# timlod/onset-fingerprinting

Hardware: AMD Instinct MI355X
Metric: frames/sec (1024-pt, hop 256, 48 kHz) detect+FFT+classify at 1/2/4/8 MI355X (higher is better)
Workload: dtype f32

## Files before the change

### include/onsetfp.h

```cpp
#ifndef ONSETFP_H
#define ONSETFP_H

#include <stdint.h>

#ifdef __cplusplus
extern "C" {
#endif

#define OFP_OK 0
#define OFP_ERR_INVALID 1
#define OFP_ERR_HIP 2
#define OFP_ERR_NODEVICE 3
#define OFP_ERR_WORKSPACE 4
#define OFP_ERR_NOCONVERGE 5

#define OFP_ABI_VERSION 3

int ofp_abi_version(void);
const char* ofp_last_error(void);
int ofp_device_count(void);
int ofp_device_check(int device, char* buf, int buflen);

#define OFP_RUNTIME_QUEUES_VAR "GPU_MAX_HW_QUEUES"
#define OFP_RUNTIME_QUEUES "16"
// ... 90 lines not shown
    int64_t mm_S;
    int64_t tu;
    int32_t sm_seg;
    int32_t merge;
    int32_t hp_early;
    int32_t hp_staged;
    int32_t hp_spread;
    int32_t hp_lines;
    int32_t ar_sym;
    int32_t ar_through;
    int32_t ar_lines;
    int32_t db_sym;
    int32_t mm_il;
    int32_t mm_through;
    int32_t ar_il;
    int32_t use_sum;
} ofp_detect_plan;
int ofp_detect_plan_query(const ofp_detector* det, int64_t n_clips, int64_t n_samples, int64_t warm, int want_rel,
                          const void* d_rel, ofp_detect_plan* out);
int ofp_detect_plan_for(const ofp_detector_params* p, const ofp_detect_tuning* t, int n_cus, int64_t n_clips,
                        int64_t n_samples, int64_t warm, int want_rel, const void* d_rel, ofp_detect_plan* out);

enum {
    OFP_CANON_LOG10 = 0,
    OFP_CANON_EXP10 = 1,
    OFP_CANON_RECT_DB = 2,
    OFP_CANON_REL_LINEAR = 3,
    OFP_CANON_AR_STEP = 4,
    OFP_CANON_MIN_STEP = 5,
    OFP_CANON_MAX_STEP = 6
};
int ofp_canon_eval(int32_t op, const float* d_x, const float* d_y, int64_t n, float p0, float p1, float p2, float* d_out,
                   void* stream);

#define OFP_DETECT_INFO_LEN 16
int ofp_detect_offline(ofp_detector* det, const float* d_x, int64_t n_clips, int64_t n_samples,
                       int64_t warm, float* d_rel, ofp_onset* d_records, int64_t cap_per_clip,
                       int64_t* d_counts, void* d_ws, int64_t ws_bytes, int64_t* h_info,
                       void* stream);

int ofp_detect_offline_enqueue(ofp_detector* det, const float* d_x, int64_t n_clips, int64_t n_samples,
                               int64_t warm, float* d_rel, ofp_onset* d_records, int64_t cap_per_clip,
                               int64_t* d_counts, void* d_ws, int64_t ws_bytes, void* stream);
int ofp_detect_offline_complete(ofp_detector* det, const float* d_x, int64_t n_clips, int64_t n_samples,
                                int64_t warm, float* d_rel, ofp_onset* d_records, int64_t cap_per_clip,
                                int64_t* d_counts, void* d_ws, int64_t ws_bytes, int64_t* h_info, void* stream);

int ofp_detect_offline_begin(ofp_detector* det, const float* d_x, int64_t n_clips, int64_t n_samples,
                             int64_t warm, void* d_ws, int64_t ws_bytes, void* stream);
int ofp_detect_offline_finish(ofp_detector* det, const float* d_x, int64_t n_clips, int64_t n_samples,
                              int64_t warm, float* d_rel, ofp_onset* d_records, int64_t cap_per_clip,
                              int64_t* d_counts, void* d_ws, int64_t ws_bytes, int64_t* h_info, void* stream);

int ofp_detect_offline_finish_enqueue(ofp_detector* det, const float* d_x, int64_t n_clips, int64_t n_samples,
                                      int64_t warm, float* d_rel, ofp_onset* d_records, int64_t cap_per_clip,
                                      int64_t* d_counts, void* d_ws, int64_t ws_bytes, void* stream);

int ofp_detect_offline_begin_input(ofp_detector* det, const float* d_x, int64_t n_clips, int64_t n_samples,
                                   int64_t warm, void* d_ws, int64_t ws_bytes, void* stream);
int ofp_detect_offline_begin_iir(ofp_detector* det, const float* d_x, int64_t n_clips, int64_t n_samples,
                                 int64_t warm, void* d_ws, int64_t ws_bytes, void* stream);
int ofp_pack_records(const ofp_onset* d_records, const int64_t* d_counts, int64_t n_clips, int64_t cap_per_clip,
                     int64_t cap_total, int32_t clip_offset, ofp_onset* d_block, void* stream);

int64_t ofp_stream_state_bytes(const ofp_detector* det);
int ofp_stream_state_init(ofp_detector* det, void* d_state, void* stream);
// ... 519 lines not shown
```

### onset_fingerprinting_amd/_lib.py

```python
import ctypes
import os
import subprocess
from pathlib import Path

_HERE = Path(__file__).resolve().parent
LIB_PATH = _HERE / "libonsetfp.so"


class OnsetFPError(RuntimeError):
    pass


class DetectorParams(ctypes.Structure):
    _fields_ = [
        ("n_channels", ctypes.c_int32),
        ("block_size", ctypes.c_int32),
        ("floor_db", ctypes.c_float),
        ("hp_enabled", ctypes.c_int32),
        ("hp_b", ctypes.c_float * 5),
        ("hp_a", ctypes.c_float * 5),
        ("fast_attack", ctypes.c_float),
        ("fast_release", ctypes.c_float),
        ("slow_attack", ctypes.c_float),
        ("slow_release", ctypes.c_float),
# ... 180 lines not shown
        ("d_audio", ctypes.c_void_p),
        ("audio_len", ctypes.c_int64),
        ("d_starts", ctypes.c_void_p),
        ("n_onsets", ctypes.c_int64),
    ]


_vp, _i32, _i64, _f32, _f64 = ctypes.c_void_p, ctypes.c_int32, ctypes.c_int64, ctypes.c_float, ctypes.c_double
_f32p_h = ctypes.POINTER(ctypes.c_float)
_long_p = ctypes.POINTER(ctypes.c_long)

SIGNATURES = {
    "ofp_abi_version": (ctypes.c_int, []),
    "ofp_last_error": (ctypes.c_char_p, []),
    "ofp_runtime_prepare": (ctypes.c_int, []),
    "ofp_device_count": (ctypes.c_int, []),
    "ofp_device_check": (ctypes.c_int, [ctypes.c_int, ctypes.c_char_p, ctypes.c_int]),
    "ar_envelope": (None, [_f32p_h, _f32p_h, _f32, _f32, ctypes.c_int, ctypes.c_int]),
    "minmax_envelope": (None, [_f32p_h, _f32p_h, _f32p_h, _f32, _f32, _f32, ctypes.c_int, ctypes.c_int]),
    "backtrack_onsets": (None, [_f32p_h, _long_p, _long_p, _f32, _f32, ctypes.c_long, ctypes.c_long,
                                ctypes.c_long, ctypes.c_long]),
    "ofp_lfilter": (ctypes.c_int, [_f32p_h, _f32p_h, _f32p_h, _f32p_h, ctypes.c_int, _f32p_h, ctypes.c_long,
                                   ctypes.c_int]),
    "ofp_detector_create": (ctypes.c_int, [ctypes.POINTER(DetectorParams), ctypes.POINTER(ctypes.c_double),
                                           ctypes.POINTER(ctypes.c_double), ctypes.POINTER(_vp)]),
    "ofp_detector_destroy": (ctypes.c_int, [_vp]),
    "ofp_detector_set_tuning": (ctypes.c_int, [_vp, ctypes.POINTER(DetectTuning)]),
    "ofp_pack_records": (ctypes.c_int, [_vp, _vp, _i64, _i64, _i64, ctypes.c_int32, _vp, _vp]),
    "ofp_detect_workspace_bytes": (_i64, [_vp, _i64, _i64, _i64]),
    "ofp_detect_plan_query": (ctypes.c_int, [_vp, _i64, _i64, _i64, ctypes.c_int, _vp, ctypes.POINTER(DetectPlan)]),
    "ofp_detect_plan_for": (ctypes.c_int, [ctypes.POINTER(DetectorParams), ctypes.POINTER(DetectTuning), ctypes.c_int,
                                           _i64, _i64, _i64, ctypes.c_int, _vp, ctypes.POINTER(DetectPlan)]),
    "ofp_canon_eval": (ctypes.c_int, [_i32, _vp, _vp, _i64, _f32, _f32, _f32, _vp, _vp]),
    "ofp_detect_offline": (ctypes.c_int, [_vp, _vp, _i64, _i64, _i64, _vp, _vp, _i64, _vp, _vp, _i64,
                                          ctypes.POINTER(_i64), _vp]),
    "ofp_detect_offline_enqueue": (ctypes.c_int, [_vp, _vp, _i64, _i64, _i64, _vp, _vp, _i64, _vp, _vp, _i64, _vp]),
    "ofp_detect_offline_complete": (ctypes.c_int, [_vp, _vp, _i64, _i64, _i64, _vp, _vp, _i64, _vp, _vp, _i64,
                                                   ctypes.POINTER(_i64), _vp]),
    "ofp_detect_offline_finish_enqueue": (ctypes.c_int, [_vp, _vp, _i64, _i64, _i64, _vp, _vp, _i64, _vp, _vp, _i64, _vp]),
    "ofp_detect_offline_begin": (ctypes.c_int, [_vp, _vp, _i64, _i64, _i64, _vp, _i64, _vp]),
    "ofp_detect_offline_finish": (ctypes.c_int, [_vp, _vp, _i64, _i64, _i64, _vp, _vp, _i64, _vp, _vp, _i64,
                                                 ctypes.POINTER(_i64), _vp]),
    "ofp_detect_offline_begin_input": (ctypes.c_int, [_vp, _vp, _i64, _i64, _i64, _vp, _i64, _vp]),
    "ofp_detect_offline_begin_iir": (ctypes.c_int, [_vp, _vp, _i64, _i64, _i64, _vp, _i64, _vp]),
    "ofp_stream_state_bytes": (_i64, [_vp]),
    "ofp_stream_state_init": (ctypes.c_int, [_vp, _vp, _vp]),
    "ofp_stream_process": (ctypes.c_int, [_vp, _vp, _vp, _i64, _i64, _i32, _i64, _vp, _vp, _i64, _vp, _vp]),
    "ofp_stream_calibrate": (ctypes.c_int, [_vp, _vp, _vp, _i64, _i64, _i64, _i64, _vp, _vp, _vp]),
    "ofp_detector_set_thresholds": (ctypes.c_int, [_vp, ctypes.POINTER(ctypes.c_double), ctypes.POINTER(ctypes.c_double)]),
    "ofp_stft_power": (ctypes.c_int, [_vp, _i64, _i64, _i32, _i32, _i32, _vp, _vp]),
    "ofp_stft_power_mel": (ctypes.c_int, [_vp, _i64, _i64, _i32, _i32, _i32, _vp, _i32, _vp, _vp, _vp, _vp, _i32, _vp,
                                          _i64, _vp]),
    "ofp_detect_planar_input": (_vp, [_vp, _i64, _i64, _i64, _vp]),
    "ofp_detect_planar_stride": (_i64, [_vp, _i64, _i64, _i64]),
    "ofp_stft_frames": (ctypes.c_int, [_vp, _i64, _i64, _i32, _vp, _vp, _vp, _vp, _vp, _i64, _i32, _i32,
                                       _vp, _vp, _vp]),
    "ofp_extract_frames": (ctypes.c_int, [_vp, _i64, _i32, _vp, _i64, _i32, _vp, _vp]),
    "ofp_mel": (ctypes.c_int, [_vp, _i64, _i32, _i32, _vp, _vp, _vp, _vp, _vp, _vp]),
    "ofp_mfcc": (ctypes.c_int, [_vp, _i64, _i32, _i32, _f32, _f32, _vp, _vp, _vp, _vp]),
    "ofp_dense": (ctypes.c_int, [_vp, _i64, _i32, _i32, _vp, _vp, _vp, _vp, _i32, _vp, _vp]),
    "ofp_mlp_create": (ctypes.c_int, [_i32, ctypes.POINTER(_i32), ctypes.POINTER(_i32), ctypes.POINTER(_vp),
                                      ctypes.POINTER(_vp), ctypes.POINTER(_vp), ctypes.POINTER(_vp),
                                      ctypes.POINTER(_vp)]),
    "ofp_mlp_destroy": (ctypes.c_int, [_vp]),
    "ofp_mlp_lds_bytes": (_i64, [_vp]),
    "ofp_mlp_forward": (ctypes.c_int, [_vp, _vp, _i64, _vp, _vp]),
# ... 263 lines not shown
```

### onset_fingerprinting_amd/csrc/ofp_canon.hip

```cpp
#include "ofp_common.h"
#include "../../include/ofp_math.h"

namespace {

using ofp::cdiv;

struct CanonArgs {
    int32_t op;
    float p0, p1, p2;
};

__global__ __launch_bounds__(256) void k_canon_eval(CanonArgs a, const float* __restrict__ x, const float* __restrict__ y,
                                                    int64_t n, float* __restrict__ out) {
    const int64_t step = (int64_t)gridDim.x * blockDim.x;
    for (int64_t i = (int64_t)blockIdx.x * blockDim.x + threadIdx.x; i < n; i += step) {
        const float xi = x[i];
        float r;
        switch (a.op) {
            case OFP_CANON_LOG10: r = ofp_log10f(xi); break;
            case OFP_CANON_EXP10: r = ofp_exp10f(xi); break;
            case OFP_CANON_RECT_DB: r = ofp_rect_db(xi, a.p0); break;
            case OFP_CANON_REL_LINEAR: r = ofp_rel_linear(xi, a.p0); break;
            case OFP_CANON_AR_STEP: r = ofp_ar_step(xi, y[i], a.p0, a.p1); break;
            case OFP_CANON_MIN_STEP: r = ofp_min_step(xi, y[i], a.p2, a.p0, a.p1); break;
            default: r = ofp_max_step(xi, y[i], a.p2, a.p0); break;
        }
        out[i] = r;
    }
}

}

extern "C" int ofp_canon_eval(int32_t op, const float* d_x, const float* d_y, int64_t n, float p0, float p1, float p2,
                              float* d_out, void* stream) {
    OFP_REQUIRE(op >= OFP_CANON_LOG10 && op <= OFP_CANON_MAX_STEP, "ofp_canon_eval: unknown op %d", (int)op);
    OFP_REQUIRE(n >= 0, "ofp_canon_eval: negative n");
    if (n == 0) return OFP_OK;
    OFP_REQUIRE(d_x && d_out, "ofp_canon_eval: NULL argument");
    const bool two = op >= OFP_CANON_AR_STEP;
    OFP_REQUIRE(!two || d_y, "ofp_canon_eval: op %d takes a second operand, d_y is NULL", (int)op);
    CanonArgs a{op, p0, p1, p2};
    if (op == OFP_CANON_MIN_STEP || op == OFP_CANON_MAX_STEP) a.p2 = ofp_ialpha(p0);
    const unsigned blocks = (unsigned)(cdiv(n, 256) < 8192 ? cdiv(n, 256) : 8192);
    hipLaunchKernelGGL(k_canon_eval, dim3(blocks), dim3(256), 0, (hipStream_t)stream, a, d_x, d_y, n, d_out);
    OFP_LAUNCH_CHECK("k_canon_eval");
    return OFP_OK;
}
```

### onset_fingerprinting_amd/csrc/ofp_detect.hip

```cpp
#include <algorithm>
#include <cstdlib>
#include <cmath>
#include <cstring>
#include <new>
#include <vector>

#include "../../include/ofp_math.h"
#include "ofp_common.h"

#include "ofp_detector.h"

#define OFP_LATENCY_BOUND_KERNEL() __builtin_amdgcn_s_setprio(3)

namespace {

using ofp::align_up;
using ofp::cdiv;

typedef float v2f __attribute__((ext_vector_type(2)));

struct Geom {
    int64_t N;
    int64_t Nm;
    int64_t n_w;
    int64_t n_wb;
    int64_t U;
    int64_t V;
    int64_t Nv;
    int32_t C, B;
};
__host__ __device__ inline int64_t hp_dst(const Geom& g, int64_t v) {
    return v < g.n_wb ? v : (v >= g.n_w ? v - g.n_w + g.n_wb : -1);
}
__host__ __device__ inline int64_t u_src(const Geom& g, int64_t u) { return u < g.n_wb ? u : u - g.n_wb; }
__host__ __device__ inline int64_t u_src_planar(const Geom& g, int64_t u) { return u < g.n_wb ? u : u - g.n_wb + g.n_w; }

template <int PB4, int OUT, bool EV, class F>
__device__ __forceinline__ void walk(const float* ip, float* op, int64_t n, int& rem, F& f) {
    auto one = [&](float x) {
        float o = f(x);
// ... 1651 lines not shown
                if (a.U[a.slot(clip, k, c, r)] == HP_EMPTY) continue;
                const uint32_t* m = a.M + a.mslot(clip, k, c, r, q);
                if (m[0] == z0 && m[1] == z1 && m[2] == z2 && m[3] == z3) {
                    joined = r;
                    break;
                }
            }
            if (joined >= 0) n_done = q + 1;
        }
    }
    if (!act) return;
    if (!whole) {
        if (sb == 0) a.ran[ci] = (int8_t)own;
        a.done[ci * a.S + sb] = 1;
        return;
    }
    if (own < 0 || a.guessed[ci]) {
        uint32_t* u = a.U + a.slot(clip, k, c, a.R);
        uint32_t* e = a.E + a.slot(clip, k, c, a.R);
        const uint32_t* ej = joined >= 0 ? a.E + a.slot(clip, k, c, joined) : nullptr;
#pragma unroll
        for (int i = 0; i < 4; ++i) {
            u[i] = xin[i];
            e[i] = ej ? ej[i] : ofp_f2u(s.z[i]);
        }
    }
    a.ran[ci] = (int8_t)a.R;
    for (int q = 0; q < n_done; ++q) a.done[ci * a.S + q] = 1;
    __threadfence();
    a.mrg[ci] = (int8_t)joined;
    if (joined >= 0) atomicAdd(a.counters + 1, 1);
}

__global__ __launch_bounds__(256) void k_rect_db(Geom g, const float* __restrict__ xt, float* __restrict__ buf,
                                                 int64_t n_chains, int from_x, float floor_db) {
    const int64_t total = n_chains * g.U;
    const int64_t tid0 = (int64_t)blockIdx.x * blockDim.x + threadIdx.x, nthr = (int64_t)gridDim.x * blockDim.x;
    if (!from_x) {
        float4* b4 = reinterpret_cast<float4*>(buf);
        const int64_t n4 = total >> 2;
        for (int64_t i = tid0; i < n4; i += nthr) {
            float4 v = b4[i];
            v.x = ofp_rect_db(v.x, floor_db);
            v.y = ofp_rect_db(v.y, floor_db);
            v.z = ofp_rect_db(v.z, floor_db);
            v.w = ofp_rect_db(v.w, floor_db);
            b4[i] = v;
        }
        for (int64_t i = (n4 << 2) + tid0; i < total; i += nthr) buf[i] = ofp_rect_db(buf[i], floor_db);
        return;
    }
    for (int64_t i = tid0; i < total; i += nthr) {
        const int64_t chain = i / g.U, u = i - chain * g.U;
        buf[i] = ofp_rect_db(xt[chain * g.Nv + u_src_planar(g, u)], floor_db);
    }
}

__global__ __launch_bounds__(64) void k_rect_db_sym(ArArgs a, float* __restrict__ buf, int64_t n_waves,
                                                    double* __restrict__ P) {
    const int64_t id = blockIdx.x;
    if (id >= n_waves) return;
    const int lane = threadIdx.x;
    const int64_t j = id % a.n_chunks;
    const int64_t chain = id / a.n_chunks;
    const int64_t base = j * a.L;
    const int64_t len = min(a.L, a.g.U - base);
    float4* xs = reinterpret_cast<float4*>(buf + chain * a.g.U + base);
    const int64_t ng = len >> 2;
    const double c = (double)a.sa, q = 1.0 - c;
    const double q2 = q * q, q4 = q2 * q2;
    double q256 = q4;
    for (int i = 0; i < 6; ++i) q256 *= q256;
    double w = c;
    for (int i = 0; i < lane; ++i) w *= q4;
    double acc = 0.0;
    auto one = [&](float4 v, int64_t g) {
        v.x = ofp_rect_db(v.x, a.floor_db);
        v.y = ofp_rect_db(v.y, a.floor_db);
        v.z = ofp_rect_db(v.z, a.floor_db);
        v.w = ofp_rect_db(v.w, a.floor_db);
        xs[ng - 1 - g] = v;
        acc += w * ((double)v.w + q * ((double)v.z + q * ((double)v.y + q * (double)v.x)));
        w *= q256;
    };
    int64_t g = lane;
    for (; g + 192 < ng; g += 256) {
        const float4 v0 = xs[ng - 1 - g], v1 = xs[ng - 1 - g - 64], v2 = xs[ng - 1 - g - 128], v3 = xs[ng - 1 - g - 192];
        __builtin_amdgcn_sched_barrier(0);
        one(v0, g);
        one(v1, g + 64);
        one(v2, g + 128);
        one(v3, g + 192);
    }
    for (; g < ng; g += 64) one(xs[ng - 1 - g], g);
    for (int o = 32; o > 0; o >>= 1) acc += __shfl_xor(acc, o);
    if (lane == 0) P[id] = acc;
}

__device__ __forceinline__ void rel_out_tile(const Geom& g, float* __restrict__ buf, float* __restrict__ rel_out,
                                             float floor_db, int TU, uint32_t* __restrict__ sum_max,
                                             uint32_t* __restrict__ sum_minv, int64_t nb, float* __restrict__ rel_warm,
                                             int planar, int64_t tile_x, float* tile) {
    const int C = g.C;
    const int S = TU + 4;
    const int64_t clip = blockIdx.y;
    const int64_t u0 = tile_x * TU;
    const int nt = (int)min<int64_t>(TU, g.U - u0);
    const int total = nt * C;
    const bool sum = sum_max != nullptr && u0 + nt > g.n_wb;
    const int64_t j0 = max<int64_t>(u0 - g.n_wb, 0) / g.B;
    const int nbt = TU / g.B + 2;
    uint32_t* s_max = reinterpret_cast<uint32_t*>(tile + (size_t)C * S);
    uint32_t* s_minv = s_max + C * nbt;
    const int lb = (g.B & (g.B - 1)) == 0 ? 31 - __clz(g.B) : -1;
    const int mbase = (int)(u0 - g.n_wb - j0 * g.B);
    if (sum) {
        for (int i = threadIdx.x; i < 2 * C * nbt; i += 256) s_max[i] = 0u;
        __syncthreads();
    }
    const bool vec = (g.U & 3) == 0 && (TU & 3) == 0 && (nt & 3) == 0 && ((g.n_wb * C) & 3) == 0 &&
                     (((int64_t)TU * C) & 3) == 0 && ((g.Nm * C) & 3) == 0;
    if (vec) {
        const int q = nt >> 2;
        const int lq = (q & (q - 1)) == 0 ? 31 - __clz(q) : -1;
        auto at = [&](int i) -> float4* {
            const int c = lq >= 0 ? i >> lq : i / q, t = (i - c * q) << 2;
            return reinterpret_cast<float4*>(buf + (clip * C + c) * g.U + u0 + t);
        };
        auto one = [&](int i, float4 v) {
            const int c = lq >= 0 ? i >> lq : i / q, t = (i - c * q) << 2;
            v.x = ofp_rel_linear(v.x, floor_db);
            v.y = ofp_rel_linear(v.y, floor_db);
            v.z = ofp_rel_linear(v.z, floor_db);
            v.w = ofp_rel_linear(v.w, floor_db);
            if (planar) *at(i) = v;
            *reinterpret_cast<float4*>(tile + c * S + t) = v;
            const int m = mbase + t;
            if (sum && m >= 0) {
                float hi = fmaxf(fmaxf(v.x, v.y), fmaxf(v.z, v.w)), lo = fminf(fminf(v.x, v.y), fminf(v.z, v.w));
                if (!(hi >= 0.0f)) hi = 0.0f;
                if (!(lo >= 0.0f)) lo = __builtin_inff();
                const int jb = lb >= 0 ? m >> lb : m / g.B;
                atomicMax(&s_max[c * nbt + jb], ofp_f2u(hi));
                atomicMax(&s_minv[c * nbt + jb], 0x7f800000u - ofp_f2u(lo));
            }
        };
        int i = threadIdx.x;
        for (; i + 768 < q * C; i += 1024) {
            const float4 v0 = *at(i), v1 = *at(i + 256), v2 = *at(i + 512), v3 = *at(i + 768);
            __builtin_amdgcn_sched_barrier(0);
            one(i, v0);
            one(i + 256, v1);
            one(i + 512, v2);
            one(i + 768, v3);
        }
        for (; i < q * C; i += 256) one(i, *at(i));
    } else {
        for (int i = threadIdx.x; i < total; i += 256) {
            const int c = i / nt, t = i - c * nt;
            float* p = buf + (clip * C + c) * g.U + u0 + t;
            const float v = ofp_rel_linear(*p, floor_db);
            if (planar) *p = v;
            tile[c * S + t] = v;
        }
    }
    __syncthreads();
    if (sum) {
        for (int i = threadIdx.x; i < C * nbt; i += 256) {
            const int c = i / nbt;
            const int64_t j = j0 + (i - c * nbt);
            if (j < nb && (s_max[i] | s_minv[i]) != 0u) {
                atomicMax(&sum_max[(clip * nb + j) * C + c], s_max[i]);
                atomicMax(&sum_minv[(clip * nb + j) * C + c], s_minv[i]);
            }
        }
    }
    if (!rel_out) return;
    float* dst = rel_out + clip * g.Nm * C;
    float* dstw = rel_warm ? rel_warm + clip * g.n_wb * C : nullptr;
    const int64_t m0 = u0 - g.n_wb;
    if (vec && (m0 >= 0 || m0 + nt <= 0) && (reinterpret_cast<uintptr_t>(rel_out) & 15u) == 0) {
        if (m0 < 0 && !dstw) return;
        float4* d4 = reinterpret_cast<float4*>(m0 < 0 ? dstw + u0 * C : dst + m0 * C);
        const int lc = (C & (C - 1)) == 0 ? 31 - __clz(C) : -1;
        for (int i = threadIdx.x; i < (total >> 2); i += 256) {
            float o[4];
#pragma unroll
            for (int e = 0; e < 4; ++e) {
                const int j = 4 * i + e;
                const int t = lc >= 0 ? j >> lc : j / C, c = j - t * C;
                o[e] = tile[c * S + t];
            }
            d4[i] = make_float4(o[0], o[1], o[2], o[3]);
        }
        return;
    }
    for (int i = threadIdx.x; i < total; i += 256) {
        const int t = i / C, c = i - t * C;
        const int64_t m = u0 + t - g.n_wb;
        if (m >= 0) dst[m * C + c] = tile[c * S + t];
        else if (dstw) dstw[(u0 + t) * C + c] = tile[c * S + t];
    }
}

__global__ __launch_bounds__(256) void k_rel_out(Geom g, float* __restrict__ buf, float* __restrict__ rel_out,
                                                 float floor_db, int TU, uint32_t* __restrict__ sum_max,
                                                 uint32_t* __restrict__ sum_minv, int64_t nb, float* __restrict__ rel_warm,
                                                 int planar, int64_t n_tiles) {
    extern __shared__ float tile[];
    for (int64_t tx = blockIdx.x; tx < n_tiles; tx += gridDim.x) {
        rel_out_tile(g, buf, rel_out, floor_db, TU, sum_max, sum_minv, nb, rel_warm, planar, tx, tile);
        __syncthreads();
    }
}

template <int CH>
__global__ __launch_bounds__(256) void k_rel_out_il(Geom g, float* __restrict__ rel, float* __restrict__ rel_warm, float floor_db,
                                                    uint32_t* __restrict__ sum_max, uint32_t* __restrict__ sum_minv,
                                                    int64_t nb, int64_t n_wu) {
    const int lane = threadIdx.x & 63;
    const int wave = __builtin_amdgcn_readfirstlane(threadIdx.x >> 6);
    const int64_t clip = blockIdx.y;
    const int n4 = g.B * (CH / 4);
    for (int64_t j = (int64_t)blockIdx.x * 4 + wave; j < n_wu + nb; j += (int64_t)gridDim.x * 4) {
        const bool in_main = j >= n_wu;
        float4* const p = in_main ? reinterpret_cast<float4*>(rel + (clip * g.Nm + (j - n_wu) * g.B) * CH)
                               : reinterpret_cast<float4*>(rel_warm + (clip * g.n_wb + j * g.B) * CH);
        float4 hi = make_float4(0.0f, 0.0f, 0.0f, 0.0f);
        const float inf = __builtin_inff();
        float4 lo = make_float4(inf, inf, inf, inf);
        auto one = [&](int i, float4 v) {
            v.x = ofp_rel_linear(v.x, floor_db);
            v.y = ofp_rel_linear(v.y, floor_db);
            v.z = ofp_rel_linear(v.z, floor_db);
            v.w = ofp_rel_linear(v.w, floor_db);
            p[i] = v;
            hi.x = fmaxf(hi.x, v.x); hi.y = fmaxf(hi.y, v.y); hi.z = fmaxf(hi.z, v.z); hi.w = fmaxf(hi.w, v.w);
            lo.x = fminf(lo.x, v.x); lo.y = fminf(lo.y, v.y); lo.z = fminf(lo.z, v.z); lo.w = fminf(lo.w, v.w);
        };
        int i = lane;
        for (; i + 192 < n4; i += 256) {
            const float4 v0 = p[i], v1 = p[i + 64], v2 = p[i + 128], v3 = p[i + 192];
            __builtin_amdgcn_sched_barrier(0);
            one(i, v0);
            one(i + 64, v1);
            one(i + 128, v2);
            one(i + 192, v3);
        }
        for (; i < n4; i += 64) one(i, p[i]);
        if (sum_max == nullptr || !in_main) continue;
#pragma unroll
        for (int o = 32; o >= CH / 4; o >>= 1) {
            hi.x = fmaxf(hi.x, __shfl_xor(hi.x, o)); hi.y = fmaxf(hi.y, __shfl_xor(hi.y, o));
            hi.z = fmaxf(hi.z, __shfl_xor(hi.z, o)); hi.w = fmaxf(hi.w, __shfl_xor(hi.w, o));
            lo.x = fminf(lo.x, __shfl_xor(lo.x, o)); lo.y = fminf(lo.y, __shfl_xor(lo.y, o));
            lo.z = fminf(lo.z, __shfl_xor(lo.z, o)); lo.w = fminf(lo.w, __shfl_xor(lo.w, o));
        }
        if (lane < CH / 4) {
            auto minv = [&](float v) { return 0x7f800000u - ofp_f2u(v >= 0.0f ? v : inf); };
            const int64_t at = (clip * nb + (j - n_wu)) * CH + 4 * lane;
            *reinterpret_cast<uint4*>(sum_max + at) = make_uint4(ofp_f2u(hi.x), ofp_f2u(hi.y), ofp_f2u(hi.z), ofp_f2u(hi.w));
            *reinterpret_cast<uint4*>(sum_minv + at) = make_uint4(minv(lo.x), minv(lo.y), minv(lo.z), minv(lo.w));
        }
    }
}

struct ScanArgs {
    Geom g;
    const float* rel;
    const float* thr_mn;
    const float* thr_mx;
    const float* on_f;
    const float* off_f;
    const double* on_d;
    int manual;
    int64_t nb, n_clips;
    int32_t* first_cross;
    int32_t* last_below;
    uint32_t* vflag;
    const uint32_t* sum_max;
    const uint32_t* sum_minv;
};
// ... 1236 lines not shown
        OFP_HIP(hipStreamSynchronize(c.stream));
        int stuck = 0;
        for (int q = 0; q < G; ++q) {
            stuck = h_flags[2 * q] + h_flags[2 * q + 1];
            rec.info[0] += 1;
            rec.info[3] += stuck;
            if (stuck == 0) break;
        }
        it += G;
        if (stuck == 0) break;
        if (l.max_passes > 0 && it > l.max_passes)
            return ofp::fail(OFP_ERR_NOCONVERGE, "hp stage: %d chains still unresolved after %d rounds", stuck, it);
    }
    return OFP_OK;
}

ArArgs ar_args(const Call& c) {
    const Layout& l = c.l;
    const auto& p = c.d->p;
    ArArgs a;
    a.g = l.g;
    a.xdb = c.xdb; a.dif = c.dif; a.rel = c.a.rel; a.rel_warm = c.rel_warm;
    a.fa = p.fast_attack; a.fr = p.fast_release; a.sa = p.slow_attack; a.sr = p.slow_release; a.floor_db = p.floor_db;
    a.L = l.ar_L; a.W = l.ar_W; a.Wc = l.ar_Wc; a.Wf = l.ar_Wf; a.n_chunks = l.ar_chunks; a.S = l.ar_S;
    a.through = l.ar_through ? 1 : 0; a.lines = l.ar_lines ? 1 : 0;
    return a;
}

int decibels(Call& c) {
    const Layout& l = c.l;
    const auto& p = c.d->p;
    const int64_t chains = c.chains();
    if (l.db_sym) {
        hipLaunchKernelGGL(k_rect_db_sym, dim3((unsigned)(chains * l.ar_chunks)), dim3(64), 0, c.stream, ar_args(c), c.xdb,
                           chains * l.ar_chunks, c.at<double>(l.o_ar_P));
        OFP_LAUNCH_CHECK("k_rect_db_sym");
    } else {
        const unsigned ew_grid = (unsigned)std::min<int64_t>(cdiv(chains * l.g.U, 256), 256 * 16);
        hipLaunchKernelGGL(k_rect_db, dim3(ew_grid), dim3(256), 0, c.stream, l.g, c.xt, c.xdb, chains, p.hp_enabled ? 0 : 1,
                           p.floor_db);
        OFP_LAUNCH_CHECK("k_rect_db");
    }
    return OFP_OK;
}

int followers(Call& c, bool host_verified) {
    const Layout& l = c.l;
    const ArArgs a = ar_args(c);
    const int64_t chains = c.chains();
    const int64_t nt = chains * l.ar_chunks;
    uint32_t* used = c.at<uint32_t>(l.o_ar_state);
    if (l.ar_sym) {
        double* P = c.at<double>(l.o_ar_P);
        if (!l.db_sym) {
            hipLaunchKernelGGL(k_ar_sym_local, dim3((unsigned)nt), dim3(64), 0, c.stream, a, nt, P);
            OFP_LAUNCH_CHECK("k_ar_sym_local");
        }
        hipLaunchKernelGGL(k_ar_sym_combine, dim3((unsigned)chains), dim3(64), 0, c.stream, a, (const double*)P, used);
        OFP_LAUNCH_CHECK("k_ar_sym_combine");
        const int64_t ntg = chains * cdiv(l.ar_chunks, l.ar_S);
        if (l.merge)
            hipLaunchKernelGGL(l.ar_il ? (l.g.C == 8 ? k_ar_warm_both<true, 8> : k_ar_warm_both<true, 4>)
                                       : (l.ar_lines ? k_ar_warm_both<true> : k_ar_warm_both<false>),
                               dim3((unsigned)cdiv(ntg, 64)), dim3(64), 0, c.stream, a, ntg, used, state_arrays(used, 2 * nt).endA);
        else
            hipLaunchKernelGGL(k_ar_warm2, dim3(2 * (unsigned)cdiv(ntg, 64)), dim3(64), 0, c.stream, a, ntg, used);
        OFP_LAUNCH_CHECK("k_ar_warm2");
// ... 581 lines not shown
```

### onset_fingerprinting_amd/detection.py

```python
import ctypes
from typing import Optional

import numpy as np
import torch
from scipy import signal as sig

from . import _lib
from ._lib import DetectorParams, DetectTuning, OnsetFPError, check

ONSET_DTYPE = np.dtype([("clip", np.int32), ("channel", np.int32), ("sample", np.int64)])


def _stream_ptr(device):
    return ctypes.c_void_p(torch.cuda.current_stream(device).cuda_stream)


def _dev(device):
    if isinstance(device, torch.device):
        return device
    return torch.device("cuda", int(device))


def _detector_params(n_signals, block_size, floor, hipass_freq, fast_ar, slow_ar, on_threshold, off_threshold,
                     cooldown, backtrack, backtrack_buffer_size, backtrack_smooth_size, sr):
# ... 209 lines not shown
    if tuning:
        bd.set_tuning(**tuning)
    out = bd.detect(xt.contiguous(), warm=warm, want_rel=want_rel)
    recs = BatchDetector.records_to_numpy(out)
    rel = out["rel"].cpu().numpy() if want_rel else None
    return recs, rel, bd.last_info


def detect_plan(n_signals, n_clips, n_samples, block_size=128, sr=96000, warm=None, want_rel=True, rel_aligned=True,
                tuning=None, n_cus=256, floor=-70.0, hipass_freq=2000.0, fast_ar=(3.0, 383.0), slow_ar=(2205.0, 2205.0),
                on_threshold=0.5, off_threshold=0.1, cooldown=1323, backtrack=False, backtrack_buffer_size=128,
                backtrack_smooth_size=5):
    p, _, _ = _detector_params(n_signals, block_size, floor, hipass_freq, fast_ar, slow_ar, on_threshold, off_threshold,
                               cooldown, backtrack, backtrack_buffer_size, backtrack_smooth_size, sr)
    t = _tuning(tuning or {})
    warm = int(0.5 * sr) if warm is None else int(warm)
    plan = _lib.DetectPlan()
    check(_lib.lib().ofp_detect_plan_for(ctypes.byref(p), ctypes.byref(t), int(n_cus), n_clips, n_samples, warm,
                                         int(bool(want_rel)), None if rel_aligned or not want_rel else 4,
                                         ctypes.byref(plan)), "ofp_detect_plan_for")
    return plan.as_dict()


CANON_OPS = {"log10": 0, "exp10": 1, "rect_db": 2, "rel_linear": 3, "ar_step": 4, "min_step": 5, "max_step": 6}


def canon_eval(op, x, y=None, p0=0.0, p1=0.0, out=None):
    assert x.is_cuda and x.dtype == torch.float32 and x.is_contiguous()
    if y is not None:
        assert y.is_cuda and y.dtype == torch.float32 and y.is_contiguous() and y.numel() == x.numel()
    if out is None:
        out = torch.empty_like(x)
    assert out.is_cuda and out.dtype == torch.float32 and out.is_contiguous() and out.numel() == x.numel()
    check(_lib.lib().ofp_canon_eval(CANON_OPS[op], x.data_ptr(), y.data_ptr() if y is not None else None, x.numel(),
                                    p0, p1, 0.0, out.data_ptr(), _stream_ptr(x.device)), "ofp_canon_eval")
    return out


def group_onsets_device(out, n_channels, max_distance=1000, min_channels=3, close_channel=None, cap_groups=None):
    L = _lib.lib()
    recs, counts = out["records"], out["counts"]
    n_clips, cap = recs.shape[0], recs.shape[1]
    cap_groups = int(cap_groups) if cap_groups is not None else cap
    ws = torch.empty(int(L.ofp_group_workspace_bytes(n_clips, cap)), dtype=torch.uint8, device=recs.device)
    groups = torch.empty((n_clips, cap_groups, n_channels), dtype=torch.int64, device=recs.device)
    n_groups = torch.zeros(n_clips, dtype=torch.int64, device=recs.device)
    check(L.ofp_group_onsets(recs.data_ptr(), cap, counts.data_ptr(), n_clips, n_channels, int(max_distance),
                             int(min_channels), -1 if close_channel is None else int(close_channel),
                             groups.data_ptr(), cap_groups, n_groups.data_ptr(), ws.data_ptr(), ws.numel(),
                             _stream_ptr(recs.device)), "ofp_group_onsets")
    return groups, n_groups


def group_windows_device(x, groups, n_groups, frame_length, pre_samples, use_min_onset=True, cap_total=None):
    if x.dim() == 2:
        x = x.unsqueeze(0)
    assert x.is_cuda and x.dtype == torch.float32 and x.is_contiguous()
    n_clips, N, C = x.shape
    cap_groups = groups.shape[1]
    assert groups.shape == (n_clips, cap_groups, C) and groups.dtype == torch.int64 and groups.is_contiguous()
    cap_total = int(cap_total) if cap_total is not None else n_clips * cap_groups
    windows = torch.empty((cap_total, C, frame_length), dtype=torch.float32, device=x.device)
    offsets = torch.empty(n_clips + 1, dtype=torch.int64, device=x.device)
    check(_lib.lib().ofp_group_windows(x.data_ptr(), n_clips, N, C, groups.data_ptr(), cap_groups, n_groups.data_ptr(),
                                  int(pre_samples), int(bool(use_min_onset)), int(frame_length), windows.data_ptr(),
                                  cap_total, offsets.data_ptr(), _stream_ptr(x.device)), "ofp_group_windows")
# ... 435 lines not shown
```

Measured before the change: 230.5 million.

## Stage log/exp lookup tables in LDS and software-pipeline elementwise dB kernels

Copies the log and exp2 lookup tables into shared memory per block and evaluates rect_db and rel_linear from those copies instead of from global/constant tables. Rewrites the elementwise loops in the rect_db and rel_out kernels with a prefetching helper that loads the next iteration before computing the current one. Also regroups k_rect_db_sym into 256-thread blocks holding four waves each. Adds an LDS-table canon_eval entry point for testing. Each block now pays a table fill and a barrier, and the double-precision polynomial work per element is unchanged.

```diff
diff --git a/include/onsetfp.h b/include/onsetfp.h
--- a/include/onsetfp.h
+++ b/include/onsetfp.h
@@ -146,6 +146,7 @@
 };
 int ofp_canon_eval(int32_t op, const float* d_x, const float* d_y, int64_t n, float p0, float p1, float p2, float* d_out,
                    void* stream);
+int ofp_canon_eval_lds(int32_t op, const float* d_x, int64_t n, float floor_db, float* d_out, void* stream);
 
 #define OFP_DETECT_INFO_LEN 16
 int ofp_detect_offline(ofp_detector* det, const float* d_x, int64_t n_clips, int64_t n_samples,
diff --git a/onset_fingerprinting_amd/_lib.py b/onset_fingerprinting_amd/_lib.py
--- a/onset_fingerprinting_amd/_lib.py
+++ b/onset_fingerprinting_amd/_lib.py
@@ -236,6 +236,7 @@
     "ofp_detect_plan_for": (ctypes.c_int, [ctypes.POINTER(DetectorParams), ctypes.POINTER(DetectTuning), ctypes.c_int,
                                            _i64, _i64, _i64, ctypes.c_int, _vp, ctypes.POINTER(DetectPlan)]),
     "ofp_canon_eval": (ctypes.c_int, [_i32, _vp, _vp, _i64, _f32, _f32, _f32, _vp, _vp]),
+    "ofp_canon_eval_lds": (ctypes.c_int, [_i32, _vp, _i64, _f32, _vp, _vp]),
     "ofp_detect_offline": (ctypes.c_int, [_vp, _vp, _i64, _i64, _i64, _vp, _vp, _i64, _vp, _vp, _i64,
                                           ctypes.POINTER(_i64), _vp]),
     "ofp_detect_offline_enqueue": (ctypes.c_int, [_vp, _vp, _i64, _i64, _i64, _vp, _vp, _i64, _vp, _vp, _i64, _vp]),
diff --git a/onset_fingerprinting_amd/csrc/ofp_canon.hip b/onset_fingerprinting_amd/csrc/ofp_canon.hip
--- a/onset_fingerprinting_amd/csrc/ofp_canon.hip
+++ b/onset_fingerprinting_amd/csrc/ofp_canon.hip
@@ -1,5 +1,6 @@
 #include "ofp_common.h"
 #include "../../include/ofp_math.h"
+#include "ofp_canon_dev.h"
 
 namespace {
 
@@ -29,6 +30,19 @@
     }
 }
 
+__global__ __launch_bounds__(256) void k_canon_eval_lds(CanonArgs a, const float* __restrict__ x, int64_t n,
+                                                        float* __restrict__ out) {
+    __shared__ ofp_canon::LogTables lg;
+    __shared__ ofp_canon::ExpTable ex;
+    ofp_canon::fill(lg);
+    ofp_canon::fill(ex);
+    const int64_t step = (int64_t)gridDim.x * blockDim.x;
+    for (int64_t i = (int64_t)blockIdx.x * blockDim.x + threadIdx.x; i < n; i += step) {
+        const float xi = x[i];
+        out[i] = a.op == OFP_CANON_RECT_DB ? ofp_canon::rect_db(xi, a.p0, lg.r, lg.t) : ofp_canon::rel_linear(xi, a.p0, ex.t);
+    }
+}
+
 }
 
 extern "C" int ofp_canon_eval(int32_t op, const float* d_x, const float* d_y, int64_t n, float p0, float p1, float p2,
@@ -46,3 +60,15 @@
     OFP_LAUNCH_CHECK("k_canon_eval");
     return OFP_OK;
 }
+
+extern "C" int ofp_canon_eval_lds(int32_t op, const float* d_x, int64_t n, float floor_db, float* d_out, void* stream) {
+    OFP_REQUIRE(op == OFP_CANON_RECT_DB || op == OFP_CANON_REL_LINEAR, "ofp_canon_eval_lds: unknown op %d", (int)op);
+    OFP_REQUIRE(n >= 0, "ofp_canon_eval_lds: negative n");
+    if (n == 0) return OFP_OK;
+    OFP_REQUIRE(d_x && d_out, "ofp_canon_eval_lds: NULL argument");
+    CanonArgs a{op, floor_db, 0.0f, 0.0f};
+    const unsigned blocks = (unsigned)(cdiv(n, 256) < 8192 ? cdiv(n, 256) : 8192);
+    hipLaunchKernelGGL(k_canon_eval_lds, dim3(blocks), dim3(256), 0, (hipStream_t)stream, a, d_x, n, d_out);
+    OFP_LAUNCH_CHECK("k_canon_eval_lds");
+    return OFP_OK;
+}
diff --git a/onset_fingerprinting_amd/csrc/ofp_canon_dev.h b/onset_fingerprinting_amd/csrc/ofp_canon_dev.h
--- /dev/null
+++ b/onset_fingerprinting_amd/csrc/ofp_canon_dev.h
@@ -0,0 +1,104 @@
+#ifndef OFP_CANON_DEV_H
+#define OFP_CANON_DEV_H
+
+#include "../../include/ofp_math.h"
+
+#pragma clang fp contract(off)
+
+namespace ofp_canon {
+
+OFP_D float log10f_from(float a, const double* log_r, const double* log_t) {
+    if (a != a) return a;
+    if (a == 0.0f) return ofp_u2f(0xff800000u);
+    if (a < 0.0f) return ofp_u2f(0x7fc00000u);
+    if (ofp_f2u(a) == 0x7f800000u) return a;
+    uint64_t u = ofp_d2u((double)a);
+    int k = (int)((u >> 52) & 0x7ff) - 1023;
+    uint64_t mant = u & 0x000fffffffffffffull;
+    int i = (int)(mant >> 45);
+    uint64_t ebits = 0x3ff0000000000000ull;
+    if (i >= 53) {
+        ebits = 0x3fe0000000000000ull;
+        k += 1;
+    }
+    double m = ofp_u2d(ebits | mant);
+    double z = m * log_r[i] - 1.0;
+    double p = -0.1;
+    p = p * z + (1.0 / 9.0);
+    p = p * z - 0.125;
+    p = p * z + (1.0 / 7.0);
+    p = p * z - (1.0 / 6.0);
+    p = p * z + 0.2;
+    p = p * z - 0.25;
+    p = p * z + (1.0 / 3.0);
+    p = p * z - 0.5;
+    p = p * z + 1.0;
+    p = p * z;
+    double r = (double)k * OFP_LOG10_2 + log_t[i];
+    r = r + p * OFP_LOG10_E;
+    return (float)r;
+}
+
+OFP_D float exp10f_from(float v, const double* exp2_t) {
+    if (v != v) return v;
+    if (v >= 39.0f) return ofp_u2f(0x7f800000u);
+    if (v <= -46.0f) return 0.0f;
+    double t = (double)v * OFP_LOG2_10;
+    double tn = t * 32.0;
+    int n = (int)(tn + (tn >= 0.0 ? 0.5 : -0.5));
+    double f = t - (double)n * 0.03125;
+    double y = f * OFP_LN2;
+    double p = 1.0 / 5040.0;
+    p = p * y + (1.0 / 720.0);
+    p = p * y + (1.0 / 120.0);
+    p = p * y + (1.0 / 24.0);
+    p = p * y + (1.0 / 6.0);
+    p = p * y + 0.5;
+    p = p * y + 1.0;
+    p = p * y + 1.0;
+    int e = n >> 5;
+    double s = ofp_u2d((uint64_t)(1023 + e) << 52);
+    double r = exp2_t[n & 31] * p;
+    r = r * s;
+    return (float)r;
+}
+
+OFP_D float rect_db(float x, float floor_db, const double* log_r, const double* log_t) {
+    float a = x + 1e-10f;
+    a = a < 0.0f ? -a : a;
+    float v = 20.0f * log10f_from(a, log_r, log_t);
+    return v < floor_db ? floor_db : v;
+}
+
+OFP_D float rel_linear(float dif, float floor_db, const double* exp2_t) {
+    float v = exp10f_from(dif / 20.0f, exp2_t) - 1e-10f;
+    float hi = -floor_db;
+    v = v < 0.0f ? 0.0f : v;
+    v = v > hi ? hi : v;
+    return v;
+}
+
+struct LogTables {
+    double r[128], t[128];
+};
+struct ExpTable {
+    double t[32];
+};
+
+OFP_D void fill(LogTables& s) {
+    const int i = threadIdx.x;
+    if (i < 128) {
+        s.r[i] = OFP_LOG_R[i];
+        s.t[i] = OFP_LOG_T[i];
+    }
+    __syncthreads();
+}
+OFP_D void fill(ExpTable& s) {
+    const int i = threadIdx.x;
+    if (i < 32) s.t[i] = OFP_EXP2_T[i];
+    __syncthreads();
+}
+
+}
+
+#endif
diff --git a/onset_fingerprinting_amd/csrc/ofp_detect.hip b/onset_fingerprinting_amd/csrc/ofp_detect.hip
--- a/onset_fingerprinting_amd/csrc/ofp_detect.hip
+++ b/onset_fingerprinting_amd/csrc/ofp_detect.hip
@@ -6,6 +6,7 @@
 #include <vector>
 
 #include "../../include/ofp_math.h"
+#include "ofp_canon_dev.h"
 #include "ofp_common.h"
 
 #include "ofp_detector.h"
@@ -1723,35 +1724,68 @@
     if (joined >= 0) atomicAdd(a.counters + 1, 1);
 }
 
+struct Quad {
+    float4 v0, v1, v2, v3;
+};
+template <class I, class Load, class Work>
+__device__ __forceinline__ void stream_trips(I i, I n, I step, Load load, Work work) {
+    if (i >= n) return;
+    auto cur = load(i);
+    for (I ni = i + step; ni < n; ni += step) {
+        const auto nxt = load(ni);
+        __builtin_amdgcn_sched_barrier(0);
+        work(i, cur);
+        cur = nxt;
+        i = ni;
+    }
+    work(i, cur);
+}
+
+__device__ __forceinline__ float4 rect_db4(float4 v, float floor_db, const ofp_canon::LogTables& tb) {
+    v.x = ofp_canon::rect_db(v.x, floor_db, tb.r, tb.t);
+    v.y = ofp_canon::rect_db(v.y, floor_db, tb.r, tb.t);
+    v.z = ofp_canon::rect_db(v.z, floor_db, tb.r, tb.t);
+    v.w = ofp_canon::rect_db(v.w, floor_db, tb.r, tb.t);
+    return v;
+}
+__device__ __forceinline__ float4 rel_linear4(float4 v, float floor_db, const ofp_canon::ExpTable& tb) {
+    v.x = ofp_canon::rel_linear(v.x, floor_db, tb.t);
+    v.y = ofp_canon::rel_linear(v.y, floor_db, tb.t);
+    v.z = ofp_canon::rel_linear(v.z, floor_db, tb.t);
+    v.w = ofp_canon::rel_linear(v.w, floor_db, tb.t);
+    return v;
+}
+
 __global__ __launch_bounds__(256) void k_rect_db(Geom g, const float* __restrict__ xt, float* __restrict__ buf,
                                                  int64_t n_chains, int from_x, float floor_db) {
+    __shared__ ofp_canon::LogTables tb;
+    ofp_canon::fill(tb);
     const int64_t total = n_chains * g.U;
     const int64_t tid0 = (int64_t)blockIdx.x * blockDim.x + threadIdx.x, nthr = (int64_t)gridDim.x * blockDim.x;
     if (!from_x) {
         float4* b4 = reinterpret_cast<float4*>(buf);
         const int64_t n4 = total >> 2;
-        for (int64_t i = tid0; i < n4; i += nthr) {
-            float4 v = b4[i];
-            v.x = ofp_rect_db(v.x, floor_db);
-            v.y = ofp_rect_db(v.y, floor_db);
-            v.z = ofp_rect_db(v.z, floor_db);
-            v.w = ofp_rect_db(v.w, floor_db);
-            b4[i] = v;
-        }
-        for (int64_t i = (n4 << 2) + tid0; i < total; i += nthr) buf[i] = ofp_rect_db(buf[i], floor_db);
+        stream_trips(tid0, n4, nthr, [&](int64_t i) { return b4[i]; },
+                     [&](int64_t i, float4 v) { b4[i] = rect_db4(v, floor_db, tb); });
+        const int64_t i = (n4 << 2) + tid0;
+        if (i < total) buf[i] = ofp_canon::rect_db(buf[i], floor_db, tb.r, tb.t);
         return;
     }
-    for (int64_t i = tid0; i < total; i += nthr) {
-        const int64_t chain = i / g.U, u = i - chain * g.U;
-        buf[i] = ofp_rect_db(xt[chain * g.Nv + u_src_planar(g, u)], floor_db);
-    }
-}
-
-__global__ __launch_bounds__(64) void k_rect_db_sym(ArArgs a, float* __restrict__ buf, int64_t n_waves,
-                                                    double* __restrict__ P) {
-    const int64_t id = blockIdx.x;
+    stream_trips(tid0, total, nthr,
+                 [&](int64_t i) {
+                     const int64_t chain = i / g.U, u = i - chain * g.U;
+                     return xt[chain * g.Nv + u_src_planar(g, u)];
+                 },
+                 [&](int64_t i, float v) { buf[i] = ofp_canon::rect_db(v, floor_db, tb.r, tb.t); });
+}
+
+__global__ __launch_bounds__(256) void k_rect_db_sym(ArArgs a, float* __restrict__ buf, int64_t n_waves,
+                                                     double* __restrict__ P) {
+    __shared__ ofp_canon::LogTables tb;
+    ofp_canon::fill(tb);
+    const int64_t id = (int64_t)blockIdx.x * 4 + __builtin_amdgcn_readfirstlane(threadIdx.x >> 6);
     if (id >= n_waves) return;
-    const int lane = threadIdx.x;
+    const int lane = threadIdx.x & 63;
     const int64_t j = id % a.n_chunks;
     const int64_t chain = id / a.n_chunks;
     const int64_t base = j * a.L;
@@ -1766,24 +1800,22 @@
     for (int i = 0; i < lane; ++i) w *= q4;
     double acc = 0.0;
     auto one = [&](float4 v, int64_t g) {
-        v.x = ofp_rect_db(v.x, a.floor_db);
-        v.y = ofp_rect_db(v.y, a.floor_db);
-        v.z = ofp_rect_db(v.z, a.floor_db);
-        v.w = ofp_rect_db(v.w, a.floor_db);
+        v = rect_db4(v, a.floor_db, tb);
         xs[ng - 1 - g] = v;
         acc += w * ((double)v.w + q * ((double)v.z + q * ((double)v.y + q * (double)v.x)));
         w *= q256;
     };
-    int64_t g = lane;
-    for (; g + 192 < ng; g += 256) {
-        const float4 v0 = xs[ng - 1 - g], v1 = xs[ng - 1 - g - 64], v2 = xs[ng - 1 - g - 128], v3 = xs[ng - 1 - g - 192];
-        __builtin_amdgcn_sched_barrier(0);
-        one(v0, g);
-        one(v1, g + 64);
-        one(v2, g + 128);
-        one(v3, g + 192);
-    }
-    for (; g < ng; g += 64) one(xs[ng - 1 - g], g);
+    const int64_t n_full = ng - lane > 192 ? (ng - lane - 193) / 256 + 1 : 0;
+    stream_trips(int64_t(lane), lane + 256 * n_full, int64_t(256),
+                 [&](int64_t g) { return Quad{xs[ng - 1 - g], xs[ng - 1 - g - 64], xs[ng - 1 - g - 128], xs[ng - 1 - g - 192]}; },
+                 [&](int64_t g, const Quad& v) {
+                     one(v.v0, g);
+                     one(v.v1, g + 64);
+                     one(v.v2, g + 128);
+                     one(v.v3, g + 192);
+                 });
+    stream_trips(lane + 256 * n_full, ng, int64_t(64), [&](int64_t g) { return xs[ng - 1 - g]; },
+                 [&](int64_t g, float4 v) { one(v, g); });
     for (int o = 32; o > 0; o >>= 1) acc += __shfl_xor(acc, o);
     if (lane == 0) P[id] = acc;
 }
@@ -1791,7 +1823,7 @@
 __device__ __forceinline__ void rel_out_tile(const Geom& g, float* __restrict__ buf, float* __restrict__ rel_out,
                                              float floor_db, int TU, uint32_t* __restrict__ sum_max,
                                              uint32_t* __restrict__ sum_minv, int64_t nb, float* __restrict__ rel_warm,
-                                             int planar, int64_t tile_x, float* tile) {
+                                             int planar, int64_t tile_x, float* tile, const ofp_canon::ExpTable& tb) {
     const int C = g.C;
     const int S = TU + 4;
     const int64_t clip = blockIdx.y;
@@ -1820,10 +1852,7 @@
         };
         auto one = [&](int i, float4 v) {
             const int c = lq >= 0 ? i >> lq : i / q, t = (i - c * q) << 2;
-            v.x = ofp_rel_linear(v.x, floor_db);
-            v.y = ofp_rel_linear(v.y, floor_db);
-            v.z = ofp_rel_linear(v.z, floor_db);
-            v.w = ofp_rel_linear(v.w, floor_db);
+            v = rel_linear4(v, floor_db, tb);
             if (planar) *at(i) = v;
             *reinterpret_cast<float4*>(tile + c * S + t) = v;
             const int m = mbase + t;
@@ -1845,15 +1874,19 @@
             one(i + 512, v2);
             one(i + 768, v3);
         }
-        for (; i < q * C; i += 256) one(i, *at(i));
+        stream_trips(i, q * C, 256, [&](int i) { return *at(i); }, [&](int i, float4 v) { one(i, v); });
     } else {
-        for (int i = threadIdx.x; i < total; i += 256) {
+        auto at = [&](int i) -> float* {
             const int c = i / nt, t = i - c * nt;
-            float* p = buf + (clip * C + c) * g.U + u0 + t;
-            const float v = ofp_rel_linear(*p, floor_db);
-            if (planar) *p = v;
-            tile[c * S + t] = v;
-        }
+            return buf + (clip * C + c) * g.U + u0 + t;
+        };
+        stream_trips((int)threadIdx.x, total, 256, [&](int i) { return *at(i); },
+                     [&](int i, float x) {
+                         const int c = i / nt, t = i - c * nt;
+                         const float v = ofp_canon::rel_linear(x, floor_db, tb.t);
+                         if (planar) *at(i) = v;
+                         tile[c * S + t] = v;
+                     });
     }
     __syncthreads();
     if (sum) {
@@ -1899,8 +1932,10 @@
                                                  uint32_t* __restrict__ sum_minv, int64_t nb, float* __restrict__ rel_warm,
                                                  int planar, int64_t n_tiles) {
     extern __shared__ float tile[];
+    __shared__ ofp_canon::ExpTable tb;
+    ofp_canon::fill(tb);
     for (int64_t tx = blockIdx.x; tx < n_tiles; tx += gridDim.x) {
-        rel_out_tile(g, buf, rel_out, floor_db, TU, sum_max, sum_minv, nb, rel_warm, planar, tx, tile);
+        rel_out_tile(g, buf, rel_out, floor_db, TU, sum_max, sum_minv, nb, rel_warm, planar, tx, tile, tb);
         __syncthreads();
     }
 }
@@ -1909,6 +1944,8 @@
 __global__ __launch_bounds__(256) void k_rel_out_il(Geom g, float* __restrict__ rel, float* __restrict__ rel_warm, float floor_db,
                                                     uint32_t* __restrict__ sum_max, uint32_t* __restrict__ sum_minv,
                                                     int64_t nb, int64_t n_wu) {
+    __shared__ ofp_canon::ExpTable tb;
+    ofp_canon::fill(tb);
     const int lane = threadIdx.x & 63;
     const int wave = __builtin_amdgcn_readfirstlane(threadIdx.x >> 6);
     const int64_t clip = blockIdx.y;
@@ -1921,10 +1958,7 @@
         const float inf = __builtin_inff();
         float4 lo = make_float4(inf, inf, inf, inf);
         auto one = [&](int i, float4 v) {
-            v.x = ofp_rel_linear(v.x, floor_db);
-            v.y = ofp_rel_linear(v.y, floor_db);
-            v.z = ofp_rel_linear(v.z, floor_db);
-            v.w = ofp_rel_linear(v.w, floor_db);
+            v = rel_linear4(v, floor_db, tb);
             p[i] = v;
             hi.x = fmaxf(hi.x, v.x); hi.y = fmaxf(hi.y, v.y); hi.z = fmaxf(hi.z, v.z); hi.w = fmaxf(hi.w, v.w);
             lo.x = fminf(lo.x, v.x); lo.y = fminf(lo.y, v.y); lo.z = fminf(lo.z, v.z); lo.w = fminf(lo.w, v.w);
@@ -1938,7 +1972,7 @@
             one(i + 128, v2);
             one(i + 192, v3);
         }
-        for (; i < n4; i += 64) one(i, p[i]);
+        stream_trips(i, n4, 64, [&](int i) { return p[i]; }, [&](int i, float4 v) { one(i, v); });
         if (sum_max == nullptr || !in_main) continue;
 #pragma unroll
         for (int o = 32; o >= CH / 4; o >>= 1) {
@@ -3241,7 +3275,7 @@
     const auto& p = c.d->p;
     const int64_t chains = c.chains();
     if (l.db_sym) {
-        hipLaunchKernelGGL(k_rect_db_sym, dim3((unsigned)(chains * l.ar_chunks)), dim3(64), 0, c.stream, ar_args(c), c.xdb,
+        hipLaunchKernelGGL(k_rect_db_sym, dim3((unsigned)cdiv(chains * l.ar_chunks, 4)), dim3(256), 0, c.stream, ar_args(c), c.xdb,
                            chains * l.ar_chunks, c.at<double>(l.o_ar_P));
         OFP_LAUNCH_CHECK("k_rect_db_sym");
     } else {
diff --git a/onset_fingerprinting_amd/detection.py b/onset_fingerprinting_amd/detection.py
--- a/onset_fingerprinting_amd/detection.py
+++ b/onset_fingerprinting_amd/detection.py
@@ -265,6 +265,10 @@
     if out is None:
         out = torch.empty_like(x)
     assert out.is_cuda and out.dtype == torch.float32 and out.is_contiguous() and out.numel() == x.numel()
+    if op.endswith("_lds"):
+        check(_lib.lib().ofp_canon_eval_lds(CANON_OPS[op[:-4]], x.data_ptr(), x.numel(), p0, out.data_ptr(),
+                                            _stream_ptr(x.device)), "ofp_canon_eval_lds")
+        return out
     check(_lib.lib().ofp_canon_eval(CANON_OPS[op], x.data_ptr(), y.data_ptr() if y is not None else None, x.numel(),
                                     p0, p1, 0.0, out.data_ptr(), _stream_ptr(x.device)), "ofp_canon_eval")
     return out
```

After: 234.8 million (median of 6 runs). 1.02x the previous value.
